# erikszasz/GaussianSplattingRegistration

Measured on AMD Instinct MI355X. Metric: Gaussians/sec through HEM level + ICP iters/sec, 2x5M-splat pair, higher is better.
Workload: dtype f32 (HEM) / f64 (ICP)

## Files before the change

### gaussiansplattingregistration_amd/_lib.py

```python
from __future__ import annotations

import ctypes as C
import os

_HERE = os.path.dirname(os.path.abspath(__file__))
LIB_PATH = os.environ.get("GSR_HIP_LIB") or os.path.join(_HERE, "csrc", "libgsr_hip.so")

GSR_OK = 0
GSR_E_INVALID = -1
GSR_E_HIP = -2
GSR_E_NO_DEVICE = -3
GSR_E_PRECONDITION = -4

GSR_RNG_GLIBC = 0
GSR_RNG_HASH = 1

GSR_ICP_ACC_LEN = 32

GSR_COMM_ID_BYTES = 128

GSR_DECOMP_REFERENCE = 0
GSR_DECOMP_EXACT = 1

ALLREDUCE_FN = C.CFUNCTYPE(C.c_int32, C.POINTER(C.c_double), C.c_int32, C.c_void_p)
# ... 75 lines not shown
    "gsr_normals_from_cov": (_i32, [_vp, _i64, _vp, _i32, _i32, _vp]),
    "gsr_normals_knn": (_i32, [_vp, _i64, _i32, _vp, _i32, _i32, _vp]),
    "gsr_cov_from_normals": (_i32, [_vp, _i64, _f64, _vp, _i32, _i32, _vp]),
    "gsr_decompose_cov": (_i32, [_vp, _i64, _i32, _vp, _vp, _vp, _i32, _i32, _vp]),
    "gsr_ply_unpack": (_i32, [_vp, _i64, _i32, C.POINTER(_i32), _i32, _vp, _vp, _vp, _vp, _vp, _vp, _vp, _i32, _vp]),
    "gsr_ply_pack": (_i32, [_vp, _vp, _vp, _vp, _vp, _vp, _i64, _i32, _vp, _i32, _vp]),
    "gsr_sh_rotation": (_i32, [_vp, _i32, _vp]),
    "gsr_model_transform": (_i32, [_vp, _i64, _i32, _i32, _vp, _vp, _vp, _vp, _vp, _vp, _vp, _vp, _i32, _i32, _vp]),
    "gsr_model_similarity": (_i32, [_vp, _i64, _i32, _i32, _vp, _vp, _vp, _vp, _vp, _vp, _vp, _vp, _vp, _vp, _i32, _i32, _vp]),
    "gsr_model_fuse": (_i32, [_vp, _vp, _i32, _vp, _vp, _vp, _vp, _i32, _i32, _vp]),
    "gsr_plane_score": (_i32, [_vp, _vp, _i64, _vp, _i32, _f32, _f32, _vp, _vp, C.POINTER(_i32), _i32, _i32, _vp]),
    "gsr_icp_solve": (_i32, [_vp, _i32, _vp, _vp]),
    "gsr_icp_get_centre": (_i32, [_vp, _vp]),
    "gsr_hybrid_search": (_i32, [_vp, _i64, _f64, _i32, _vp, _vp, _i32, _i32, _vp]),
    "gsr_fpfh": (_i32, [_vp, _vp, _i64, _f64, _i32, _vp, _i32, _i32, _vp]),
    "gsr_feature_match": (_i32, [_vp, _i64, _vp, _i64, _i32, _i32, _vp, C.POINTER(_i64), C.POINTER(_i32), _vp, _vp, _i32, _i32, _vp]),
    "gsr_ransac_correspondence": (_i32, [_vp, _i64, _vp, _i64, _vp, _vp, _vp, _i64, _vp, _vp, _i32, _i32, _vp]),
    "gsr_fgr_tuple_test": (_i32, [_vp, _i64, _vp, _i64, _vp, _i64, _vp, _vp, C.POINTER(_i64), C.POINTER(_i64), _i32, _i32, _vp]),
    "gsr_fgr_optimize": (_i32, [_vp, _i64, _vp, _i64, _vp, _i64, _vp, _vp, _i32, _i32, _vp]),
    "gsr_posegraph_optimize": (_i32, [_i32, _vp, _i32, _vp, _vp, _vp, _vp, _vp]),
    "gsr_raster_create": (_i32, [C.POINTER(_vp), _i32, _vp]),
    "gsr_raster_destroy": (_i32, [_vp]),
    "gsr_raster_render": (_i32, [_vp, _i64, _i32, _i32, _vp, _vp, _vp, _vp, _vp, C.POINTER(_f32), _f32, _f32, _f32, _f32, _i32, _i32, C.POINTER(_f32), _f32,
                                 _vp, _vp, _vp]),
    "gsr_raster_get_timing": (_i32, [_vp, C.POINTER(_f32)]),
    "gsr_image_metrics": (_i32, [_vp, _vp, _i32, _i32, _i32, C.POINTER(_f64), _i32, _vp]),
}
TEST_HOOKS = {
    "gsr_debug_logf": (_i32, [_vp, _i64, _vp, _i32]),
    "gsr_debug_kld": (_i32, [_vp, _vp, _vp, _vp, _i64, _vp, _i32]),
    "gsr_debug_kl_gate": (_i32, [_vp, _vp, _vp, _i64, _f32, _vp, _vp, _vp, _i32]),
    "gsr_debug_stage1": (_i32, [_vp, _vp, _vp, _vp, _i64, _f32, _vp, _vp, _vp, _vp, _vp, _vp, _i32]),
    "gsr_debug_ransac_sample": (_i32, [_u64, _i64, _i64, _i64, _i32, _vp]),
}

_lib = None


class HemLevelReport(C.Structure):
    _fields_ = [("offset_rows", C.c_int64), ("rows", C.c_int64), ("dropped", C.c_int64), ("rng_position", C.c_uint64),
                ("stats", C.c_int64 * 8), ("stats_ex", C.c_int64 * 8), ("phase_ms", C.c_float * 8), ("kernel_ms", C.c_float * 8)]


class IcpEntry(C.Structure):
    _fields_ = [("src_xyz", C.c_void_p), ("ns", C.c_int64), ("tgt_xyz", C.c_void_p), ("tgt_normals", C.c_void_p), ("nt", C.c_int64),
                ("max_corr", C.c_double), ("max_iter", C.c_int32), ("reserved", C.c_int32)]


class IcpEntryResult(C.Structure):
    _fields_ = [("init_T", C.c_double * 16), ("T", C.c_double * 16), ("fitness", C.c_double), ("inlier_rmse", C.c_double),
                ("iterations", C.c_int32), ("evaluations", C.c_int32), ("ms_build", C.c_float), ("ms_iters", C.c_float)]


class RansacParams(C.Structure):
    _fields_ = [("kind", C.c_int32), ("ransac_n", C.c_int32), ("max_corr", C.c_double), ("max_iteration", C.c_int64),
                ("confidence", C.c_double), ("seed", C.c_uint64), ("batch", C.c_int32), ("n_checkers", C.c_int32),
                ("checker_kind", C.c_int32 * 4), ("checker_param", C.c_double * 4)]


class RansacResult(C.Structure):
    _fields_ = [("T", C.c_double * 16), ("fitness", C.c_double), ("inlier_rmse", C.c_double), ("best_index", C.c_int64),
                ("n_evaluated", C.c_int64), ("n_valid", C.c_int64), ("exit_index", C.c_int64)]


class FgrOptions(C.Structure):
    _fields_ = [("division_factor", C.c_double), ("use_absolute_scale", C.c_int32), ("decrease_mu", C.c_int32),
# ... 74 lines not shown
```

### gaussiansplattingregistration_amd/csrc/gsr_test_hooks.h

```cpp
#ifndef GSR_TEST_HOOKS_H
#define GSR_TEST_HOOKS_H
#include <stdint.h>
#ifdef __cplusplus
extern "C" {
#endif
int32_t gsr_debug_logf(const float* x, int64_t n, float* out, int32_t device);
int32_t gsr_debug_kld(const float* child_mean, const float* child_cov6, const float* parent_mean,
                      const float* parent_cov6, int64_t n, float* out, int32_t device);
int32_t gsr_debug_kl_gate(const float* s2, const float* det_c, const float* det_p, int64_t n, float thr, uint8_t* reject,
                          float* fast_log, uint8_t* need_exact, int32_t device);
int32_t gsr_debug_stage1(const float* parent_mean, const float* parent_cov6, const float* child_mean, const float* child_cov6, int64_t n,
                         float kld_thr, uint8_t* parent_regular, uint8_t* child_regular, uint8_t* white, uint8_t* reject, float* T1,
                         uint8_t* clip_on, int32_t device);
int32_t gsr_debug_ransac_sample(uint64_t seed, int64_t k0, int64_t count, int64_t m, int32_t n, int32_t* out);
#ifdef __cplusplus
}
#endif
#endif
```

### gaussiansplattingregistration_amd/csrc/icp.hip

```cpp
#include "gsr_common.h"
#include "gsr_normals.h"
#include "gsr_solve.h"
#include "gsr_features.h"
#include "gsr_oneshot.h"
#include "gsr_prims.h"

#include <float.h>
#include <math.h>
#include <stdlib.h>
#include <string.h>
#include <vector>

namespace gsr {
#ifndef GSR_ICP_MERGE_BS
#define GSR_ICP_MERGE_BS 1024
#define GSR_ICP_MERGE_IPT 4
#endif
using icp_merge_cfg = rocprim::merge_sort_config<512, GSR_ICP_MERGE_BS, GSR_ICP_MERGE_IPT, 128, 128, 4>;
using icp_sort_cfg = rocprim::radix_sort_config<rocprim::default_config, icp_merge_cfg,
                                                rocprim::radix_sort_onesweep_config<rocprim::kernel_config<1024, 16>, rocprim::kernel_config<1024, 16>, 11,
                                                                                    rocprim::block_radix_rank_algorithm::match>>;

#ifndef ICP_CELL_FLOOR_DIV
#define ICP_CELL_FLOOR_DIV 64.0
#endif
struct IcpGrid {
    double ox, oy, oz, inv_c, c;
    double cx, cy, cz;
    int gx, gy, gz, ncells;
    int rings;
    double bx0, by0, bz0, bx1, by1, bz1;
};

__device__ __forceinline__ int icp_cell(double v, double o, double inv_c, int g) {
    double t = (v - o) * inv_c;
    t = fmin(fmax(t, 0.0), (double)(g - 1));
    return (int)t;
}

__global__ __launch_bounds__(256) void k_icp_bbox(int64_t n, const float* __restrict__ xyz, float* __restrict__ bbox_part) {
    float mn[3] = {FLT_MAX, FLT_MAX, FLT_MAX}, mx[3] = {-FLT_MAX, -FLT_MAX, -FLT_MAX};
    for (int64_t i = (int64_t)blockIdx.x * blockDim.x + threadIdx.x; i < n; i += (int64_t)gridDim.x * blockDim.x) {
        float x = xyz[3 * i], y = xyz[3 * i + 1], z = xyz[3 * i + 2];
        if (fabsf(x) <= FLT_MAX && fabsf(y) <= FLT_MAX && fabsf(z) <= FLT_MAX) {
            mn[0] = fminf(mn[0], x); mx[0] = fmaxf(mx[0], x);
            mn[1] = fminf(mn[1], y); mx[1] = fmaxf(mx[1], y);
            mn[2] = fminf(mn[2], z); mx[2] = fmaxf(mx[2], z);
        }
    }
    __shared__ float s_mn[4][3], s_mx[4][3];
    for (int k = 0; k < 3; ++k)
        for (int o = 32; o > 0; o >>= 1) { mn[k] = fminf(mn[k], __shfl_xor(mn[k], o)); mx[k] = fmaxf(mx[k], __shfl_xor(mx[k], o)); }
    if ((threadIdx.x & 63) == 0)
        for (int k = 0; k < 3; ++k) { s_mn[threadIdx.x >> 6][k] = mn[k]; s_mx[threadIdx.x >> 6][k] = mx[k]; }
    __syncthreads();
    if (threadIdx.x < 3) {
        const int k = threadIdx.x;
        float a = s_mn[0][k], b = s_mx[0][k];
        for (int w = 1; w < 4; ++w) { a = fminf(a, s_mn[w][k]); b = fmaxf(b, s_mx[w][k]); }
        bbox_part[6 * blockIdx.x + k] = a;
        bbox_part[6 * blockIdx.x + 3 + k] = b;
    }
}
__global__ __launch_bounds__(256) void k_icp_bbox_reduce(int nblocks, const float* __restrict__ part, float* __restrict__ bbox) {
// ... 120 lines not shown

struct ColorArgs {
    const double* t_int;
    const double* t_grad;
    const double* s_int;
    double sqrt_lg, sqrt_lp;
};

__device__ __forceinline__ void icp_scan_span(const int* __restrict__ cellStart, const float4* __restrict__ Tq, int first, int last,
                                              double px, double py, double pz, double& bd, int& best, unsigned& best_i) {
    const int s = cellStart[first], e = cellStart[last + 1];
    for (int j = s; j < e; ++j) {
        const float4 q = Tq[j];
        const double dx = px - (double)q.x, dy = py - (double)q.y, dz = pz - (double)q.z;
        const double d2 = dx * dx + dy * dy + dz * dz;
        const unsigned qi = __float_as_uint(q.w);
        if (d2 < bd || (d2 == bd && qi < best_i)) { bd = d2; best = j; best_i = qi; }
    }
}

__device__ __forceinline__ double icp_slab_dist(double v, double o, double c, int k, double eps, int g) {
    const double lo = o + (double)k * c, hi = o + (double)(k + 1) * c;
    const double d = ((v < lo && k > 0) ? lo - v : ((v > hi && k < g - 1) ? v - hi : 0.0)) * 0.999999999 - eps;
    return d > 0.0 ? d : 0.0;
}

__device__ __forceinline__ void icp_consider(const float4 q, int j, double px, double py, double pz, double& bd, int& best, unsigned& best_i) {
    const double dx = px - (double)q.x, dy = py - (double)q.y, dz = pz - (double)q.z;
    const double d2 = dx * dx + dy * dy + dz * dz;
    const unsigned qi = __float_as_uint(q.w);
    if (d2 < bd || (d2 == bd && qi < best_i)) { bd = d2; best = j; best_i = qi; }
}

#define ICP_BLOCK_CROWDED 24
#ifndef ICP_ROW_BATCH
#define ICP_ROW_BATCH 4
#endif
template <int BLOCK>
__device__ __forceinline__ int icp_nearest(const IcpGrid& g, const int* __restrict__ cellStart,
                                           const float4* __restrict__ Tq, double px, double py, double pz, double& best_d2,
                                           double bound2 = 1.0 / 0.0) {
    int best = -1;
    unsigned best_i = 0xffffffffu;
    double bd = bound2;
    if (!(px == px) || !(py == py) || !(pz == pz)) { best_d2 = 1.0 / 0.0; return -1; }
    {
        const double ex = fmax(fmax(g.bx0 - px, px - g.bx1), 0.0), ey = fmax(fmax(g.by0 - py, py - g.by1), 0.0), ez = fmax(fmax(g.bz0 - pz, pz - g.bz1), 0.0);
        if ((ex * ex + ey * ey + ez * ez) * 0.999999999 >= bound2) { best_d2 = bound2; return -1; }
    }
    const int cx = icp_cell(px, g.ox, g.inv_c, g.gx), cy = icp_cell(py, g.oy, g.inv_c, g.gy), cz = icp_cell(pz, g.oz, g.inv_c, g.gz);
    const double eps = 1e-13 * (fabs(px) + fabs(py) + fabs(pz) + fabs(g.ox) + fabs(g.oy) + fabs(g.oz) + g.c * (double)(g.gx + g.gy + g.gz));
    int r0 = 0;
    if (BLOCK == 1 && g.rings >= 1) {
        int rs[9], re[9];
        const int xa = cx - 1 > 0 ? cx - 1 : 0, xb = cx + 1 < g.gx - 1 ? cx + 1 : g.gx - 1;
#pragma unroll
        for (int t = 0; t < 9; ++t) {
            const int z = cz + t / 3 - 1, y = cy + t % 3 - 1;
            const bool ok = z >= 0 && z < g.gz && y >= 0 && y < g.gy;
            const int rowbase = ok ? (z * g.gy + y) * g.gx : 0;
            rs[t] = ok ? cellStart[rowbase + xa] : 0;
            re[t] = ok ? cellStart[rowbase + xb + 1] : 0;
        }
        {
        constexpr int order9[9] = {4, 1, 3, 5, 7, 0, 2, 6, 8};
#pragma unroll
        for (int tt = 0; tt < 9; ++tt) {
            const int t = order9[tt];
            if (t != 4 && re[t] - rs[t] > ICP_BLOCK_CROWDED) {
                const double dzb = icp_slab_dist(pz, g.oz, g.c, cz + t / 3 - 1, eps, g.gz), dyb = icp_slab_dist(py, g.oy, g.c, cy + t % 3 - 1, eps, g.gy);
                if (dzb * dzb + dyb * dyb > bd) continue;
            }
            for (int j = rs[t]; j < re[t]; j += ICP_ROW_BATCH) {
                const int l = re[t] - 1;
                int jj[ICP_ROW_BATCH];
                float4 qq[ICP_ROW_BATCH];
#pragma unroll
                for (int b = 0; b < ICP_ROW_BATCH; ++b) { jj[b] = j + b < l ? j + b : l; qq[b] = Tq[jj[b]]; }
#pragma unroll
                for (int b = 0; b < ICP_ROW_BATCH; ++b) icp_consider(qq[b], jj[b], px, py, pz, bd, best, best_i);
            }
        }
        }
    }
    if (BLOCK && g.rings >= 1) {
        double reach = 1.0 / 0.0;
        if (cx - 1 > 0) reach = fmin(reach, px - (g.ox + (double)(cx - 1) * g.c));
        if (cx + 1 < g.gx - 1) reach = fmin(reach, (g.ox + (double)(cx + 2) * g.c) - px);
        if (cy - 1 > 0) reach = fmin(reach, py - (g.oy + (double)(cy - 1) * g.c));
        if (cy + 1 < g.gy - 1) reach = fmin(reach, (g.oy + (double)(cy + 2) * g.c) - py);
        if (cz - 1 > 0) reach = fmin(reach, pz - (g.oz + (double)(cz - 1) * g.c));
        if (cz + 1 < g.gz - 1) reach = fmin(reach, (g.oz + (double)(cz + 2) * g.c) - pz);
        reach = reach * 0.999999999 - eps;
        reach = reach > 0.0 ? reach : 0.0;
        if (bd < reach * reach) { best_d2 = bd; return best; }
        r0 = 2;
    }
    for (int r = r0; r <= g.rings; ++r) {
        for (int dz = -r; dz <= r; ++dz) {
            const int z = cz + dz;
            if (z < 0 || z >= g.gz) continue;
            const int adz = dz < 0 ? -dz : dz;
            const double dzb = icp_slab_dist(pz, g.oz, g.c, z, eps, g.gz);
            for (int dy = -r; dy <= r; ++dy) {
                const int y = cy + dy;
                if (y < 0 || y >= g.gy) continue;
                const int ady = dy < 0 ? -dy : dy;
                const double dyb = icp_slab_dist(py, g.oy, g.c, y, eps, g.gy);
                const double rem = bd - dyb * dyb - dzb * dzb;
                if (rem < 0.0) continue;
                int xlo = 0, xhi = g.gx - 1;
                if (rem < 1e300) {
                    const double hx = (double)(sqrtf((float)rem) * 1.0001f) + eps + 1e-30;
                    xlo = icp_cell(px - hx, g.ox, g.inv_c, g.gx);
                    xhi = icp_cell(px + hx, g.ox, g.inv_c, g.gx);
// ... 36 lines not shown
    IcpRange r;
    r.row = L < nb ? L : -1;
    r.lo = (int64_t)L * ppb;
    r.hi = r.lo + ppb < ns ? r.lo + ppb : ns;
    return r;
}

struct IcpState;
__device__ __forceinline__ bool icp_state_done(const IcpState* st);
__device__ __forceinline__ void icp_state_T(const IcpState* st, double T[12]);

template <bool FROM_STATE, int BLOCK>
__global__ __launch_bounds__(256) void k_icp_nn(int64_t ns, const float* __restrict__ src, Xform X, const IcpState* __restrict__ st,
                                                IcpGrid g, const int* __restrict__ cellStart, const float4* __restrict__ Tq,
                                                double max_corr2, int* __restrict__ nn_j, int nb_logical) {
    double T[12];
    if (FROM_STATE) {
        if (icp_state_done(st)) return;
        icp_state_T(st, T);
    } else {
#pragma unroll
        for (int i = 0; i < 12; ++i) T[i] = X.m[i];
    }
    const IcpRange rg = icp_block_range(ns, nb_logical < 0 ? -nb_logical : nb_logical, nb_logical > 0);
    if (rg.row < 0) return;
    for (int64_t i = rg.lo + threadIdx.x; i < rg.hi; i += blockDim.x) {
        const double x = (double)src[3 * i], y = (double)src[3 * i + 1], z = (double)src[3 * i + 2];
        const double px = T[0] * x + T[1] * y + T[2] * z + T[3];
        const double py = T[4] * x + T[5] * y + T[6] * z + T[7];
        const double pz = T[8] * x + T[9] * y + T[10] * z + T[11];
        double d2;
        const int j = icp_nearest<BLOCK>(g, cellStart, Tq, px, py, pz, d2, max_corr2);
        nn_j[i] = (j >= 0 && d2 < max_corr2) ? j : -1;
    }
}

__device__ __forceinline__ double icp_weight(int loss, double k, double r) {
    switch (loss) {
        case GSR_LOSS_TUKEY: { double t = fmin(1.0, fabs(r) / k); double u = 1.0 - t * t; return u * u; }
        case GSR_LOSS_CAUCHY: { double t = r / k; return 1.0 / (1.0 + t * t); }
        case GSR_LOSS_GM: { double t = k + r * r; return k / (t * t); }
        case GSR_LOSS_HUBER: { double e = fabs(r); return k / fmax(e, k); }
        default: return 1.0;
    }
}

__host__ __device__ static void sym_eig3(double a00, double a01, double a02, double a11, double a12, double a22, double V[3][3], double lam[3]) {
    double A[3][3] = {{a00, a01, a02}, {a01, a11, a12}, {a02, a12, a22}};
    for (int i = 0; i < 3; ++i) for (int j = 0; j < 3; ++j) V[i][j] = i == j ? 1.0 : 0.0;
    for (int sweep = 0; sweep < 30; ++sweep) {
        const double off = A[0][1] * A[0][1] + A[0][2] * A[0][2] + A[1][2] * A[1][2];
        const double dg = A[0][0] * A[0][0] + A[1][1] * A[1][1] + A[2][2] * A[2][2];
        if (!(off > 1e-40 * dg)) break;
#pragma unroll
        for (int p = 0; p < 2; ++p)
#pragma unroll
            for (int q = p + 1; q < 3; ++q) {
                if (A[p][q] == 0.0) continue;
                const double theta = (A[q][q] - A[p][p]) / (2.0 * A[p][q]);
                const double t = (theta >= 0 ? 1.0 : -1.0) / (fabs(theta) + sqrt(theta * theta + 1.0));
                const double c = 1.0 / sqrt(t * t + 1.0), sn = t * c;
#pragma unroll
                for (int k = 0; k < 3; ++k) { const double x = A[k][p], y = A[k][q]; A[k][p] = c * x - sn * y; A[k][q] = sn * x + c * y; }
#pragma unroll
                for (int k = 0; k < 3; ++k) { const double x = A[p][k], y = A[q][k]; A[p][k] = c * x - sn * y; A[q][k] = sn * x + c * y; }
#pragma unroll
// ... 615 lines not shown
    icp_step_solve(&s_x[0][0], s_st, st);
}

__global__ __launch_bounds__(1024) void k_icp_reduce(int nblocks, const double* __restrict__ partials, const IcpState* __restrict__ st,
                                                     double* __restrict__ out) {
    const int lane = threadIdx.x & 63, wv = threadIdx.x >> 6;
    const bool done = st->done != 0;
    for (int k = wv; k < GSR_ICP_ACC_LEN; k += 16) {
        double s = 0.0;
        if (!done)
            for (int b = lane; b < nblocks; b += 64) s += partials[(int64_t)b * GSR_ICP_ACC_LEN + k];
        for (int o = 32; o > 0; o >>= 1) s += __shfl_xor(s, o);
        if (lane == 0) out[k] = s;
    }
}

}

using namespace gsr;

struct gsr_icp_ctx {
    int device = 0;
    hipStream_t stream = nullptr;
    IcpGrid grid;
    bool have_target = false, have_normals = false, have_source = false;
    int64_t nt = 0, ns = 0, ns_global = 0;
    double max_corr = 0;
    DevBuf src_raw, src_order, state, nn_j, Tc, Sc, stage_cov, Ti, Tg, Si;
    bool have_tcov = false, have_scov = false, have_tcol = false, have_scol = false;
    double lambda_geometric = 0.968;
    bool src_sorted = false;
    bool device_loop = true;
    bool block_search = true;
    bool xcd_ranges = true;
    gsr_comm* comm = nullptr;
    PinnedBlock host_rb;
    unsigned long long rb_seq = 0;
    int nn_kernel = -1;
    int nn_mode() const { return nn_kernel >= 0 ? (nn_kernel ? 2 : 0) : (ns >= 400000 ? 2 : 0); }
    double cell_target = 2.0;
    DevBuf hist;
    bool robust_box = false;
    bool robust_allowed = true;
    DevBuf bbox, keys, idx, skeys, order, cellStart, Tq, Tn, stage_xyz, stage_nrm, src, partials, acc_dev, rocprim_tmp, corr_idx, corr_d2;
    gsr_allreduce_fn allreduce = nullptr;
    void* allreduce_user = nullptr;
    gsr_allreduce_dev64_fn allreduce_dev = nullptr;
    void* allreduce_dev_user = nullptr;
    Event e0, e1, eb0, eb1;
    bool defer_sync = false;
    bool build_pending = false;
    float ms_build = 0, ms_iter = 0;
    int n_iter_kernels = 0;
    int max_cells = 1 << 25;
    int nblocks = 768;
    ~gsr_icp_ctx() { (void)hipSetDevice(device); }
};

namespace {

inline int icp_blocks(int64_t ns, int cap) {
    if (ns <= 0) return 1;
    const int64_t ppb = ((ns + cap - 1) / cap + 255) / 256 * 256;
    return (int)((ns + ppb - 1) / ppb);
}
inline int nn_grid1(int64_t ns) { return icp_blocks(ns, 16384); }
// ... 117 lines not shown
static int32_t icp_fetch(gsr_icp_ctx* c, const void* dev, void* out, size_t bytes) {
    hipStream_t st = c->stream;
    unsigned* const host_rb = c->host_rb.as<unsigned>();
    if (!host_rb || bytes > 1024 || (bytes & 3)) {
        GSR_HIP(hipMemcpyAsync(out, dev, bytes, hipMemcpyDeviceToHost, st));
        GSR_HIP(hipStreamSynchronize(st));
        return GSR_OK;
    }
    const unsigned long long seq = ++c->rb_seq;
    unsigned long long* flag = reinterpret_cast<unsigned long long*>(host_rb + 256);
    hipLaunchKernelGGL(k_icp_publish, dim3(1), dim3(64), 0, st, (const unsigned*)dev, (int)(bytes >> 2), host_rb, flag, seq);
    GSR_HIP(hipGetLastError());
    GSR_TRY(wait_host_flag(st, flag, seq, true));
    memcpy(out, (const void*)host_rb, bytes);
    return GSR_OK;
}

int32_t gsr_icp_create(gsr_icp_ctx** out, int32_t device, void* stream) {
    if (!out) return fail(GSR_E_INVALID, "gsr_icp_create: out is NULL");
    *out = nullptr;
    int ndev = 0;
    if (hipGetDeviceCount(&ndev) != hipSuccess || ndev <= 0)
        return fail(GSR_E_NO_DEVICE, "gsr_icp_create: no HIP device visible (this backend has no CPU fallback)");
    if (device < 0 || device >= ndev) return fail(GSR_E_INVALID, "gsr_icp_create: device %d out of range", device);
    GSR_HIP(hipSetDevice(device));
    gsr_icp_ctx* c = new gsr_icp_ctx();
    c->device = device;
    c->stream = (hipStream_t)stream;
    if (c->e0.create() != hipSuccess || c->e1.create() != hipSuccess || c->eb0.create() != hipSuccess || c->eb1.create() != hipSuccess) {
        delete c; return fail(GSR_E_HIP, "hipEventCreate failed");
    }
    if (const char* e = getenv("GSR_ICP_DEVICE_LOOP")) c->device_loop = atoi(e) != 0;
    if (const char* e = getenv("GSR_ICP_BLOCK_SEARCH")) c->block_search = atoi(e) != 0;
    if (const char* e = getenv("GSR_ICP_XCD")) c->xcd_ranges = atoi(e) != 0;
    if (const char* e = getenv("GSR_ICP_ROBUST_BOX")) c->robust_allowed = atoi(e) != 0;
    if (const char* e = getenv("GSR_ICP_BLOCKS")) { int v = atoi(e); if (v >= 1 && v <= 65536) c->nblocks = v; }
    bool poll = true;
    if (const char* e = getenv("GSR_ICP_RB_POLL")) poll = atoi(e) != 0;
    if (!poll || c->host_rb.alloc(1024 + 64) != hipSuccess) (void)hipGetLastError();
    if (const char* e = getenv("GSR_ICP_NN_KERNEL")) c->nn_kernel = atoi(e);
    if (const char* e = getenv("GSR_ICP_CELL_TARGET")) { double v = atof(e); if (v > 0.01 && v < 1000) c->cell_target = v; }
    if (const char* e = getenv("GSR_ICP_MAX_CELLS")) { int v = atoi(e); if (v >= 1024) c->max_cells = v; }
    *out = c;
    return GSR_OK;
}

int32_t gsr_icp_destroy(gsr_icp_ctx* c) {
    delete c;
    return GSR_OK;
}

int32_t gsr_icp_set_target(gsr_icp_ctx* c, const float* xyz, const double* normals, int64_t n, double max_corr, int32_t on_device) {
    if (!c) return fail(GSR_E_INVALID, "gsr_icp_set_target: NULL context");
    if (!(max_corr > 0)) return fail(GSR_E_PRECONDITION, "max_correspondence_distance must be > 0 (got %g)", max_corr);
    if (n <= 0 || !xyz) return fail(GSR_E_PRECONDITION, "gsr_icp_set_target: empty target cloud");
    if (n >= ((int64_t)1 << 31) - 1) return fail(GSR_E_INVALID, "gsr_icp_set_target: n too large");
    GSR_HIP(hipSetDevice(c->device));
    hipStream_t st = c->stream;
    GSR_HIP(hipEventRecord(c->eb0, st));
    const float* dxyz = xyz;
    const double* dnrm = normals;
    if (!on_device) {
        GSR_TRY(c->stage_xyz.reserve((size_t)n * 12));
        GSR_HIP(hipMemcpyAsync(c->stage_xyz.p, xyz, (size_t)n * 12, hipMemcpyHostToDevice, st));
        dxyz = c->stage_xyz.as<float>();
        if (normals) {
// ... 14 lines not shown
    GSR_TRY(icp_fetch(c, c->bbox.p, hb, 13 * 4));
    const float raw_box[6] = {hb[0], hb[1], hb[2], hb[3], hb[4], hb[5]};
    c->robust_box = hb[12] != 0.0f && c->robust_allowed;
    if (c->robust_box) {
        GSR_HIP(hipMemsetAsync(c->hist.p, 0, 3 * ICP_HIST_BINS * 4, st));
        hipLaunchKernelGGL(k_icp_hist, dim3(nbb > 512 ? 512 : nbb), dim3(256), 0, st, n, dxyz, c->bbox.as<float>() + 6, c->hist.as<unsigned>());
        hipLaunchKernelGGL(k_icp_trim, dim3(1), dim3(64), 0, st, c->hist.as<unsigned>(), c->bbox.as<float>() + 6, c->bbox.as<float>(), c->bbox.as<float>() + 12);
        GSR_TRY(icp_fetch(c, c->bbox.p, hb, 6 * 4));
    }
    double mn[3], mx[3];
    for (int k = 0; k < 3; ++k) { mn[k] = hb[k]; mx[k] = hb[3 + k]; }
    IcpGrid g;
    if (!(mx[0] >= mn[0])) { mn[0] = mn[1] = mn[2] = 0; mx[0] = mx[1] = mx[2] = 0; }
    double cell;
    {
        const double ex = mx[0] - mn[0], ey = mx[1] - mn[1], ez = mx[2] - mn[2];
        const double emax = fmax(ex, fmax(ey, ez)), eps = emax * 1e-6 + 1e-30;
        cell = cbrt((ex + eps) * (ey + eps) * (ez + eps) * c->cell_target / (double)n);
        if (!(cell > 0)) cell = max_corr;
        if (cell < max_corr / ICP_CELL_FLOOR_DIV) cell = max_corr / ICP_CELL_FLOOR_DIV;
    }
    GSR_TRY(c->keys.reserve(n * 4)); GSR_TRY(c->idx.reserve(n * 4)); GSR_TRY(c->skeys.reserve(n * 4)); GSR_TRY(c->order.reserve(n * 4));
    for (;;) {
        double fx = floor((mx[0] - mn[0]) / cell) + 1, fy = floor((mx[1] - mn[1]) / cell) + 1, fz = floor((mx[2] - mn[2]) / cell) + 1;
        if (fx * fy * fz <= (double)c->max_cells) { g.gx = (int)fx; g.gy = (int)fy; g.gz = (int)fz; break; }
        cell *= 1.2599210498948732;
    }
    g.ox = mn[0]; g.oy = mn[1]; g.oz = mn[2];
    g.c = cell; g.inv_c = 1.0 / cell;
    g.cx = 0.5 * (mn[0] + mx[0]); g.cy = 0.5 * (mn[1] + mx[1]); g.cz = 0.5 * (mn[2] + mx[2]);
    g.ncells = g.gx * g.gy * g.gz;
    g.rings = (int)ceil(max_corr / cell);
    if (g.rings < 1) g.rings = 1;
    g.bx0 = raw_box[0]; g.by0 = raw_box[1]; g.bz0 = raw_box[2]; g.bx1 = raw_box[3]; g.by1 = raw_box[4]; g.bz1 = raw_box[5];
    if (!(raw_box[3] >= raw_box[0])) { g.bx0 = g.by0 = g.bz0 = -1.0 / 0.0; g.bx1 = g.by1 = g.bz1 = 1.0 / 0.0; }
    hipLaunchKernelGGL(k_icp_keys, dim3(stride_grid(n)), dim3(256), 0, st, n, dxyz, g, c->keys.as<unsigned>(), c->idx.as<unsigned>());
    int bits = 1;
    while (bits < 32 && ((int64_t)1 << bits) < g.ncells) ++bits;
    GSR_TRY(sort_pairs_by_key<icp_sort_cfg>(c->rocprim_tmp, st, c->keys.as<unsigned>(), c->skeys.as<unsigned>(), c->idx.as<unsigned>(),
                                            c->order.as<unsigned>(), (size_t)n, 0u, (unsigned)bits));
    GSR_TRY(c->cellStart.reserve(((size_t)g.ncells + 1) * 4));
    hipLaunchKernelGGL(k_icp_cell_starts, dim3(stride_grid(n)), dim3(256), 0, st, n, c->skeys.as<unsigned>(), (int64_t)g.ncells, c->cellStart.as<int>());
    c->grid = g;
    GSR_TRY(c->Tq.reserve((size_t)n * 16));
    if (normals) GSR_TRY(c->Tn.reserve((size_t)n * 24));
    hipLaunchKernelGGL(k_icp_gather_target, dim3(stride_grid(n)), dim3(256), 0, st, n, c->order.as<unsigned>(), dxyz, dnrm,
                       c->Tq.as<float4>(), normals ? c->Tn.as<double>() : (double*)nullptr);
    GSR_HIP(hipEventRecord(c->eb1, st));
    if (c->defer_sync) c->build_pending = true;
    else {
        GSR_HIP(hipStreamSynchronize(st));
        (void)hipEventElapsedTime(&c->ms_build, c->eb0, c->eb1);
        c->build_pending = false;
    }
    GSR_HIP(hipGetLastError());
    c->nt = n; c->max_corr = max_corr; c->have_target = true; c->have_normals = normals != nullptr;
    c->have_tcov = false; c->have_scov = false; c->have_tcol = false; c->have_scol = false;
    c->have_source = false;
    return GSR_OK;
}

int32_t gsr_icp_set_source(gsr_icp_ctx* c, const float* xyz, int64_t n, int32_t on_device) {
    if (!c) return fail(GSR_E_INVALID, "gsr_icp_set_source: NULL context");
    if (n < 0 || (n > 0 && !xyz)) return fail(GSR_E_PRECONDITION, "gsr_icp_set_source: empty source cloud");
    if (n >= ((int64_t)1 << 31) - 1) return fail(GSR_E_INVALID, "gsr_icp_set_source: n too large");
    GSR_HIP(hipSetDevice(c->device));
    hipStream_t st = c->stream;
    GSR_TRY(c->src.reserve((size_t)(n > 0 ? n : 1) * 12));
// ... 208 lines not shown
        return GSR_OK;
    }
    double T[16], acc[GSR_ICP_ACC_LEN], update[16];
    memcpy(T, init_T, sizeof(T));
    GSR_TRY(run_accumulate(c, T, kind, loss, k, acc, true));
    const double nsg = (double)(c->ns_global > 0 ? c->ns_global : c->ns);
    double fit = acc[0] > 0 ? acc[0] / nsg : 0.0, rmse = acc[0] > 0 ? sqrt(acc[1] / acc[0]) : 0.0;
    int it = 0;
    for (; it < max_iter; ++it) {
        const double ctr[3] = {c->grid.cx, c->grid.cy, c->grid.cz};
        estimate_update(ctr, kind, acc, update);
        mat4_mul(update, T, T);
        GSR_TRY(run_accumulate(c, T, kind, loss, k, acc, true));
        const double fit2 = acc[0] > 0 ? acc[0] / nsg : 0.0, rmse2 = acc[0] > 0 ? sqrt(acc[1] / acc[0]) : 0.0;
        const bool stop = fabs(fit - fit2) < rel_fitness && fabs(rmse - rmse2) < rel_rmse;
        fit = fit2; rmse = rmse2;
        if (stop) { ++it; break; }
    }
    memcpy(out_T, T, sizeof(T));
    if (fitness) *fitness = fit;
    if (inlier_rmse) *inlier_rmse = rmse;
    if (iterations) *iterations = it;
    return GSR_OK;
}

int32_t gsr_icp_correspondences(gsr_icp_ctx* c, const double* T, int64_t* idx, double* d2) {
    if (!c || !T || !idx || !d2) return fail(GSR_E_INVALID, "gsr_icp_correspondences: NULL argument");
    if (!c->have_target || !c->have_source) return fail(GSR_E_INVALID, "icp: target and source must be set first");
    GSR_HIP(hipSetDevice(c->device));
    GSR_TRY(c->corr_idx.reserve((size_t)c->ns * 8)); GSR_TRY(c->corr_d2.reserve((size_t)c->ns * 8));
    Xform X;
    for (int i = 0; i < 12; ++i) X.m[i] = T[i];
    GSR_TRY(c->nn_j.reserve((size_t)c->ns * 4));
    launch_icp_nn<false>(c, c->stream, X, (const IcpState*)nullptr, c->max_corr * c->max_corr, false);
    hipLaunchKernelGGL(k_icp_correspond, dim3(stride_grid(c->ns)), dim3(256), 0, c->stream, c->ns, c->src.as<float>(), X, c->nn_j.as<int>(),
                       c->Tq.as<float4>(), c->src_sorted ? c->src_order.as<unsigned>() : (const unsigned*)nullptr, c->corr_idx.as<int64_t>(),
                       c->corr_d2.as<double>());
    GSR_HIP(hipMemcpyAsync(idx, c->corr_idx.p, (size_t)c->ns * 8, hipMemcpyDeviceToHost, c->stream));
    GSR_HIP(hipMemcpyAsync(d2, c->corr_d2.p, (size_t)c->ns * 8, hipMemcpyDeviceToHost, c->stream));
    GSR_HIP(hipStreamSynchronize(c->stream));
    return GSR_OK;
}

int32_t gsr_icp_information(gsr_icp_ctx* c, const double* T, double* info36, int64_t* n_corr) {
    if (!c || !T || !info36) return fail(GSR_E_INVALID, "gsr_icp_information: NULL argument");
    if (!c->have_target || !c->have_source) return fail(GSR_E_INVALID, "gsr_icp_information: target and source must be set first");
    if (c->comm || c->allreduce || c->allreduce_dev)
        return fail(GSR_E_INVALID, "gsr_icp_information: one process, one GPU -- this context has a communicator or an all-reduce callback installed "
                                   "(the sums of a source shard are not the pair's information matrix)");
    for (int i = 0; i < 16; ++i)
        if (!(fabs(T[i]) <= DBL_MAX)) return fail(GSR_E_INVALID, "gsr_icp_information: T[%d] is not finite", i);
    GSR_HIP(hipSetDevice(c->device));
    hipStream_t st = c->stream;
    Xform X;
    for (int i = 0; i < 12; ++i) X.m[i] = T[i];
    const int nb = icp_blocks(c->ns, c->nblocks);
    GSR_TRY(c->partials.reserve((size_t)nb * GSR_ICP_ACC_LEN * 8));
    GSR_TRY(c->acc_dev.reserve(GSR_ICP_ACC_LEN * 8));
    GSR_HIP(hipMemsetAsync(c->partials.p, 0, (size_t)nb * GSR_ICP_ACC_LEN * 8, st));
    const double mc2 = c->max_corr * c->max_corr;
    const int* nnj = nullptr;
    if (c->nn_mode()) {
        GSR_TRY(c->nn_j.reserve((size_t)c->ns * 4));
        launch_icp_nn<false>(c, st, X, (const IcpState*)nullptr, mc2, false);
        nnj = c->nn_j.as<int>();
    }
    hipLaunchKernelGGL(k_icp_information, dim3(nb), dim3(256), 0, st, c->ns, c->src.as<float>(), X, c->grid, c->cellStart.as<int>(), nnj, c->Tq.as<float4>(),
                       mc2, c->partials.as<double>());
    hipLaunchKernelGGL(k_icp_finalize, dim3(ICP_INFO_NACC), dim3(64), 0, st, nb, c->partials.as<double>(), c->acc_dev.as<double>());
    double a[ICP_INFO_NACC];
    GSR_HIP(hipMemcpyAsync(a, c->acc_dev.p, sizeof(a), hipMemcpyDeviceToHost, st));
    GSR_HIP(hipStreamSynchronize(st));
    const double n = a[0], mx = a[1], my = a[2], mz = a[3];
    const double nxy = 0.0 - a[5], nxz = 0.0 - a[6], nyz = 0.0 - a[8];
    const double A[3][3] = {{a[7] + a[9], nxy, nxz}, {nxy, a[4] + a[9], nyz}, {nxz, nyz, a[4] + a[7]}};
    const double Mx[3][3] = {{0.0, 0.0 - mz, my}, {mz, 0.0, 0.0 - mx}, {0.0 - my, mx, 0.0}};
// ... 249 lines not shown
```

Before: 577.8 million.

## Add f32 screening pass to ICP nearest-neighbour search with certified error bounds

Adds a first pass to the ICP nearest-neighbour search that computes distances in f32 and tracks the best and second-best candidates. If a rigorous rounding-error bound shows the f32 winner cannot be overtaken, that single candidate is confirmed in f64 and the full f64 scan is skipped. Otherwise the existing f64 search runs. The aim is to replace most f64 distance arithmetic, which is slow on this GPU, with f32. The risk is that ambiguous points pay for both passes, and the extra registers may lower occupancy. A debug hook is added to report the screen's decisions.

Result: slower. 569.7 million (-1.4%).

```diff
diff --git a/gaussiansplattingregistration_amd/_lib.py b/gaussiansplattingregistration_amd/_lib.py
--- a/gaussiansplattingregistration_amd/_lib.py
+++ b/gaussiansplattingregistration_amd/_lib.py
@@ -131,6 +131,7 @@
     "gsr_debug_kl_gate": (_i32, [_vp, _vp, _vp, _i64, _f32, _vp, _vp, _vp, _i32]),
     "gsr_debug_stage1": (_i32, [_vp, _vp, _vp, _vp, _i64, _f32, _vp, _vp, _vp, _vp, _vp, _vp, _i32]),
     "gsr_debug_ransac_sample": (_i32, [_u64, _i64, _i64, _i64, _i32, _vp]),
+    "gsr_debug_icp_search": (_i32, [_vp, _vp, _i32, _i32, _vp, _vp, _vp, _vp, _vp, C.POINTER(_i64)]),
 }
 
 _lib = None
diff --git a/gaussiansplattingregistration_amd/csrc/gsr_test_hooks.h b/gaussiansplattingregistration_amd/csrc/gsr_test_hooks.h
--- a/gaussiansplattingregistration_amd/csrc/gsr_test_hooks.h
+++ b/gaussiansplattingregistration_amd/csrc/gsr_test_hooks.h
@@ -13,6 +13,9 @@
                          float kld_thr, uint8_t* parent_regular, uint8_t* child_regular, uint8_t* white, uint8_t* reject, float* T1,
                          uint8_t* clip_on, int32_t device);
 int32_t gsr_debug_ransac_sample(uint64_t seed, int64_t k0, int64_t count, int64_t m, int32_t n, int32_t* out);
+struct gsr_icp_ctx;
+int32_t gsr_debug_icp_search(struct gsr_icp_ctx* c, const double* T, int32_t block, int32_t screen, int64_t* idx, double* d2, float* m1,
+                             float* m2, uint8_t* decided, int64_t* n_undecided);
 #ifdef __cplusplus
 }
 #endif
diff --git a/gaussiansplattingregistration_amd/csrc/icp.hip b/gaussiansplattingregistration_amd/csrc/icp.hip
--- a/gaussiansplattingregistration_amd/csrc/icp.hip
+++ b/gaussiansplattingregistration_amd/csrc/icp.hip
@@ -29,7 +29,9 @@
     double cx, cy, cz;
     int gx, gy, gz, ncells;
     int rings;
+    int screen;
     double bx0, by0, bz0, bx1, by1, bz1;
+    double bmax;
 };
 
 __device__ __forceinline__ int icp_cell(double v, double o, double inv_c, int g) {
@@ -216,6 +218,14 @@
     if (d2 < bd || (d2 == bd && qi < best_i)) { bd = d2; best = j; best_i = qi; }
 }
 
+__device__ __forceinline__ double icp_screen_err(float d, double delta) {
+    return 2.0 * ((double)sqrtf(d) * 1.000001) * delta + delta * delta + 0x1p-21 * (double)d + 1e-37;
+}
+__device__ __forceinline__ double icp_screen_delta(const IcpGrid& g, double px, double py, double pz) {
+    return 3.4641016151377553 * 0x1p-24 * fmax(fmax(fmax(fabs(px), fabs(py)), fabs(pz)), g.bmax);
+}
+struct IcpScreenInfo { float m1, m2; int state; };
+
 #define ICP_BLOCK_CROWDED 24
 #ifndef ICP_ROW_BATCH
 #define ICP_ROW_BATCH 4
@@ -223,7 +233,7 @@
 template <int BLOCK>
 __device__ __forceinline__ int icp_nearest(const IcpGrid& g, const int* __restrict__ cellStart,
                                            const float4* __restrict__ Tq, double px, double py, double pz, double& best_d2,
-                                           double bound2 = 1.0 / 0.0) {
+                                           double bound2 = 1.0 / 0.0, IcpScreenInfo* info = nullptr) {
     int best = -1;
     unsigned best_i = 0xffffffffu;
     double bd = bound2;
@@ -246,8 +256,54 @@
             rs[t] = ok ? cellStart[rowbase + xa] : 0;
             re[t] = ok ? cellStart[rowbase + xb + 1] : 0;
         }
-        {
         constexpr int order9[9] = {4, 1, 3, 5, 7, 0, 2, 6, 8};
+        bool decided = false;
+        if (g.screen) {
+            const float pfx = (float)px, pfy = (float)py, pfz = (float)pz;
+            const double delta = icp_screen_delta(g, px, py, pz);
+            const float inf = __builtin_inff();
+            float m1 = inf, m2 = inf;
+            int j1 = 0;
+#pragma unroll
+            for (int tt = 0; tt < 9; ++tt) {
+                const int t = order9[tt];
+                if (t != 4 && re[t] - rs[t] > ICP_BLOCK_CROWDED) {
+                    const double dzb = icp_slab_dist(pz, g.oz, g.c, cz + t / 3 - 1, eps, g.gz), dyb = icp_slab_dist(py, g.oy, g.c, cy + t % 3 - 1, eps, g.gy);
+                    const double ub = m1 < inf ? fmin(bound2, (double)m1 + icp_screen_err(m1, delta)) : bound2;
+                    if (dzb * dzb + dyb * dyb > ub) continue;
+                }
+                for (int j = rs[t]; j < re[t]; j += ICP_ROW_BATCH) {
+                    const int l = re[t] - 1;
+                    float4 qq[ICP_ROW_BATCH];
+#pragma unroll
+                    for (int b = 0; b < ICP_ROW_BATCH; ++b) qq[b] = Tq[j + b < l ? j + b : l];
+#pragma unroll
+                    for (int b = 0; b < ICP_ROW_BATCH; ++b) {
+                        float sx = pfx - qq[b].x, sy = pfy - qq[b].y, sz = pfz - qq[b].z;
+                        asm("" : "+v"(sx), "+v"(sy), "+v"(sz));
+                        float d = __builtin_fmaf(sz, sz, __builtin_fmaf(sy, sy, sx * sx));
+                        d = j + b > l ? inf : d;
+                        m2 = fminf(m2, fmaxf(d, m1));
+                        j1 = d < m1 ? j + b : j1;
+                        m1 = fminf(m1, d);
+                    }
+                }
+            }
+            int rows = 0;
+#pragma unroll
+            for (int t = 0; t < 9; ++t) rows += re[t] - rs[t];
+            if (rows == 0) decided = true;
+            else if (m1 < inf) {
+                const double hi1 = (double)m1 + icp_screen_err(m1, delta);
+                const double lo2 = m2 < inf ? (double)m2 - icp_screen_err(m2, delta) : 3e38;
+                if (hi1 < lo2) {
+                    decided = true;
+                    icp_consider(Tq[j1], j1, px, py, pz, bd, best, best_i);
+                }
+            }
+            if (info) { info->m1 = m1; info->m2 = m2; info->state = decided ? 1 : 2; }
+        }
+        if (!decided) {
 #pragma unroll
         for (int tt = 0; tt < 9; ++tt) {
             const int t = order9[tt];
@@ -367,6 +423,29 @@
         double d2;
         const int j = icp_nearest<BLOCK>(g, cellStart, Tq, px, py, pz, d2, max_corr2);
         nn_j[i] = (j >= 0 && d2 < max_corr2) ? j : -1;
+    }
+}
+
+template <int BLOCK>
+__global__ __launch_bounds__(256) void k_icp_search_debug(int64_t ns, const float* __restrict__ src, Xform X, IcpGrid g, const int* __restrict__ cellStart,
+                                                          const float4* __restrict__ Tq, double max_corr2, const unsigned* __restrict__ src_order,
+                                                          int64_t* __restrict__ idx, double* __restrict__ d2_out, float* __restrict__ m1, float* __restrict__ m2,
+                                                          unsigned char* __restrict__ decided, unsigned long long* __restrict__ n_undecided) {
+    for (int64_t i = (int64_t)blockIdx.x * blockDim.x + threadIdx.x; i < ns; i += (int64_t)gridDim.x * blockDim.x) {
+        const double x = (double)src[3 * i], y = (double)src[3 * i + 1], z = (double)src[3 * i + 2];
+        const double px = X.m[0] * x + X.m[1] * y + X.m[2] * z + X.m[3];
+        const double py = X.m[4] * x + X.m[5] * y + X.m[6] * z + X.m[7];
+        const double pz = X.m[8] * x + X.m[9] * y + X.m[10] * z + X.m[11];
+        IcpScreenInfo info = {__builtin_inff(), __builtin_inff(), 0};
+        double d2;
+        const int j = icp_nearest<BLOCK>(g, cellStart, Tq, px, py, pz, d2, max_corr2, &info);
+        const bool ok = j >= 0 && d2 < max_corr2;
+        const int64_t o = src_order ? (int64_t)src_order[i] : i;
+        idx[o] = ok ? (int64_t)__float_as_uint(Tq[j].w) : -1;
+        d2_out[o] = ok ? d2 : 1.0 / 0.0;
+        m1[o] = info.m1; m2[o] = info.m2;
+        decided[o] = info.state == 1 ? 1 : 0;
+        if (info.state == 2) atomicAdd(n_undecided, 1ull);
     }
 }
 
@@ -1048,6 +1127,7 @@
     bool src_sorted = false;
     bool device_loop = true;
     bool block_search = true;
+    bool f32_screen = true;
     bool xcd_ranges = true;
     gsr_comm* comm = nullptr;
     PinnedBlock host_rb;
@@ -1231,6 +1311,7 @@
     }
     if (const char* e = getenv("GSR_ICP_DEVICE_LOOP")) c->device_loop = atoi(e) != 0;
     if (const char* e = getenv("GSR_ICP_BLOCK_SEARCH")) c->block_search = atoi(e) != 0;
+    if (const char* e = getenv("GSR_ICP_F32_SCREEN")) c->f32_screen = atoi(e) != 0;
     if (const char* e = getenv("GSR_ICP_XCD")) c->xcd_ranges = atoi(e) != 0;
     if (const char* e = getenv("GSR_ICP_ROBUST_BOX")) c->robust_allowed = atoi(e) != 0;
     if (const char* e = getenv("GSR_ICP_BLOCKS")) { int v = atoi(e); if (v >= 1 && v <= 65536) c->nblocks = v; }
@@ -1311,8 +1392,10 @@
     g.ncells = g.gx * g.gy * g.gz;
     g.rings = (int)ceil(max_corr / cell);
     if (g.rings < 1) g.rings = 1;
+    g.screen = c->f32_screen ? 1 : 0;
     g.bx0 = raw_box[0]; g.by0 = raw_box[1]; g.bz0 = raw_box[2]; g.bx1 = raw_box[3]; g.by1 = raw_box[4]; g.bz1 = raw_box[5];
     if (!(raw_box[3] >= raw_box[0])) { g.bx0 = g.by0 = g.bz0 = -1.0 / 0.0; g.bx1 = g.by1 = g.bz1 = 1.0 / 0.0; }
+    g.bmax = fmax(fmax(fmax(fabs(g.bx0), fabs(g.bx1)), fmax(fabs(g.by0), fabs(g.by1))), fmax(fabs(g.bz0), fabs(g.bz1)));
     hipLaunchKernelGGL(k_icp_keys, dim3(stride_grid(n)), dim3(256), 0, st, n, dxyz, g, c->keys.as<unsigned>(), c->idx.as<unsigned>());
     int bits = 1;
     while (bits < 32 && ((int64_t)1 << bits) < g.ncells) ++bits;
@@ -1597,6 +1680,50 @@
     return GSR_OK;
 }
 
+int32_t gsr_debug_icp_search(gsr_icp_ctx* c, const double* T, int32_t block, int32_t screen, int64_t* idx, double* d2, float* m1, float* m2,
+                             uint8_t* decided, int64_t* n_undecided) {
+    if (!c || !T || !idx || !d2 || !m1 || !m2 || !decided || !n_undecided) return fail(GSR_E_INVALID, "gsr_debug_icp_search: NULL argument");
+    if (!c->have_target || !c->have_source) return fail(GSR_E_INVALID, "gsr_debug_icp_search: target and source must be set first");
+    GSR_HIP(hipSetDevice(c->device));
+    hipStream_t st = c->stream;
+    const size_t n = (size_t)c->ns;
+    *n_undecided = 0;
+    if (n == 0) return GSR_OK;
+    DevBuf out;
+    GSR_TRY(out.reserve(n * 25 + 8));
+    char* const base = out.as<char>();
+    int64_t* const d_idx = (int64_t*)base;
+    double* const d_d2 = (double*)(base + n * 8);
+    float* const d_m1 = (float*)(base + n * 16);
+    float* const d_m2 = (float*)(base + n * 20);
+    unsigned long long* const d_cnt = (unsigned long long*)(base + n * 24);
+    unsigned char* const d_dec = (unsigned char*)(base + n * 24 + 8);
+    GSR_HIP(hipMemsetAsync(d_cnt, 0, 8, st));
+    Xform X;
+    for (int i = 0; i < 12; ++i) X.m[i] = T[i];
+    IcpGrid g = c->grid;
+    g.screen = screen ? 1 : 0;
+    const unsigned* order = c->src_sorted ? c->src_order.as<unsigned>() : (const unsigned*)nullptr;
+    const double mc2 = c->max_corr * c->max_corr;
+    if (block)
+        hipLaunchKernelGGL(k_icp_search_debug<1>, dim3(stride_grid(c->ns)), dim3(256), 0, st, c->ns, c->src.as<float>(), X, g, c->cellStart.as<int>(),
+                           c->Tq.as<float4>(), mc2, order, d_idx, d_d2, d_m1, d_m2, d_dec, d_cnt);
+    else
+        hipLaunchKernelGGL(k_icp_search_debug<0>, dim3(stride_grid(c->ns)), dim3(256), 0, st, c->ns, c->src.as<float>(), X, g, c->cellStart.as<int>(),
+                           c->Tq.as<float4>(), mc2, order, d_idx, d_d2, d_m1, d_m2, d_dec, d_cnt);
+    GSR_HIP(hipGetLastError());
+    unsigned long long cnt = 0;
+    GSR_HIP(hipMemcpyAsync(idx, d_idx, n * 8, hipMemcpyDeviceToHost, st));
+    GSR_HIP(hipMemcpyAsync(d2, d_d2, n * 8, hipMemcpyDeviceToHost, st));
+    GSR_HIP(hipMemcpyAsync(m1, d_m1, n * 4, hipMemcpyDeviceToHost, st));
+    GSR_HIP(hipMemcpyAsync(m2, d_m2, n * 4, hipMemcpyDeviceToHost, st));
+    GSR_HIP(hipMemcpyAsync(decided, d_dec, n, hipMemcpyDeviceToHost, st));
+    GSR_HIP(hipMemcpyAsync(&cnt, d_cnt, 8, hipMemcpyDeviceToHost, st));
+    GSR_HIP(hipStreamSynchronize(st));
+    *n_undecided = (int64_t)cnt;
+    return GSR_OK;
+}
+
 int32_t gsr_icp_information(gsr_icp_ctx* c, const double* T, double* info36, int64_t* n_corr) {
     if (!c || !T || !info36) return fail(GSR_E_INVALID, "gsr_icp_information: NULL argument");
     if (!c->have_target || !c->have_source) return fail(GSR_E_INVALID, "gsr_icp_information: target and source must be set first");
```

## Flatten 3x3 row walk into single loop with batch spill across rows

Applied to the files above, without the earlier changes.

Replaces the nested per-row loop of the nine neighbouring cell rows in the block nearest-neighbour search with a single flattened loop. The non-empty row ranges are staged in shared memory, and leftover batch slots can spill into the next short row, so fewer ICP_ROW_BATCH lanes are wasted on clamped duplicates and warp divergence across rows drops. Crowded rows are still pruned by slab distance. Separately, the correspondence entry point now enables block search when it is configured and the grid has enough rings. This adds shared memory use (a 9x256 int2 array) and assumes a block size of at most 256.

Result: no change. 580.5 million before, 577.1 million after (-0.6%).

```diff
diff --git a/gaussiansplattingregistration_amd/csrc/icp.hip b/gaussiansplattingregistration_amd/csrc/icp.hip
--- a/gaussiansplattingregistration_amd/csrc/icp.hip
+++ b/gaussiansplattingregistration_amd/csrc/icp.hip
@@ -235,7 +235,8 @@
     const int cx = icp_cell(px, g.ox, g.inv_c, g.gx), cy = icp_cell(py, g.oy, g.inv_c, g.gy), cz = icp_cell(pz, g.oz, g.inv_c, g.gz);
     const double eps = 1e-13 * (fabs(px) + fabs(py) + fabs(pz) + fabs(g.ox) + fabs(g.oy) + fabs(g.oz) + g.c * (double)(g.gx + g.gy + g.gz));
     int r0 = 0;
-    if (BLOCK == 1 && g.rings >= 1) {
+    if constexpr (BLOCK == 1) if (g.rings >= 1) {
+        __shared__ int2 s_rows[9][256];
         int rs[9], re[9];
         const int xa = cx - 1 > 0 ? cx - 1 : 0, xb = cx + 1 < g.gx - 1 ? cx + 1 : g.gx - 1;
 #pragma unroll
@@ -246,25 +247,59 @@
             rs[t] = ok ? cellStart[rowbase + xa] : 0;
             re[t] = ok ? cellStart[rowbase + xb + 1] : 0;
         }
-        {
         constexpr int order9[9] = {4, 1, 3, 5, 7, 0, 2, 6, 8};
+        unsigned rows = 0;
+        int nrows = 0;
 #pragma unroll
         for (int tt = 0; tt < 9; ++tt) {
             const int t = order9[tt];
-            if (t != 4 && re[t] - rs[t] > ICP_BLOCK_CROWDED) {
-                const double dzb = icp_slab_dist(pz, g.oz, g.c, cz + t / 3 - 1, eps, g.gz), dyb = icp_slab_dist(py, g.oy, g.c, cy + t % 3 - 1, eps, g.gy);
-                if (dzb * dzb + dyb * dyb > bd) continue;
+            if (re[t] > rs[t]) {
+                s_rows[nrows][threadIdx.x] = make_int2(rs[t], re[t]);
+                rows |= 1u << tt;
+                ++nrows;
             }
-            for (int j = rs[t]; j < re[t]; j += ICP_ROW_BATCH) {
-                const int l = re[t] - 1;
-                int jj[ICP_ROW_BATCH];
-                float4 qq[ICP_ROW_BATCH];
-#pragma unroll
-                for (int b = 0; b < ICP_ROW_BATCH; ++b) { jj[b] = j + b < l ? j + b : l; qq[b] = Tq[jj[b]]; }
-#pragma unroll
-                for (int b = 0; b < ICP_ROW_BATCH; ++b) icp_consider(qq[b], jj[b], px, py, pz, bd, best, best_i);
+        }
+        int j = 0, e = 0, jn = 0, en = 0, off = 0, lim = 0, k = 0;
+        bool spill = false;
+        if (nrows > 0) { const int2 r = s_rows[0][threadIdx.x]; jn = r.x; en = r.y; k = 1; }
+        for (;;) {
+            while (j >= e && jn < en) {
+                bool skip = false;
+                if (en - jn > ICP_BLOCK_CROWDED) {
+                    const int tt = __ffs((int)rows) - 1;
+                    if (tt != 0) {
+                        const int t = (int)((0x86207531u >> (4 * (tt - 1))) & 15u);
+                        const double dzb = icp_slab_dist(pz, g.oz, g.c, cz + t / 3 - 1, eps, g.gz), dyb = icp_slab_dist(py, g.oy, g.c, cy + t % 3 - 1, eps, g.gy);
+                        skip = dzb * dzb + dyb * dyb > bd;
+                    }
+                }
+                rows &= rows - 1;
+                j = jn + (spill ? j - e : 0);
+                j = (skip || j > en) ? en : j;
+                e = en;
+                jn = en = 0;
+                if (k < nrows) { const int2 r = s_rows[k][threadIdx.x]; jn = r.x; en = r.y; ++k; }
+#ifdef ICP_WALK_NOSPILL
+                spill = false;
+#else
+                spill = jn < en && en - jn <= ICP_BLOCK_CROWDED;
+#endif
+                off = spill ? jn - e : 0;
+                lim = spill ? en - 1 : e - 1;
             }
-        }
+            if (j >= e) break;
+            int jj[ICP_ROW_BATCH];
+            float4 qq[ICP_ROW_BATCH];
+#pragma unroll
+            for (int b = 0; b < ICP_ROW_BATCH; ++b) {
+                int i = j + b;
+                if (i >= e) { i += off; i = i < lim ? i : lim; }
+                jj[b] = i;
+                qq[b] = Tq[i];
+            }
+#pragma unroll
+            for (int b = 0; b < ICP_ROW_BATCH; ++b) icp_consider(qq[b], jj[b], px, py, pz, bd, best, best_i);
+            j += ICP_ROW_BATCH;
         }
     }
     if (BLOCK && g.rings >= 1) {
@@ -1587,7 +1622,7 @@
     Xform X;
     for (int i = 0; i < 12; ++i) X.m[i] = T[i];
     GSR_TRY(c->nn_j.reserve((size_t)c->ns * 4));
-    launch_icp_nn<false>(c, c->stream, X, (const IcpState*)nullptr, c->max_corr * c->max_corr, false);
+    launch_icp_nn<false>(c, c->stream, X, (const IcpState*)nullptr, c->max_corr * c->max_corr, c->block_search && c->grid.rings >= 2);
     hipLaunchKernelGGL(k_icp_correspond, dim3(stride_grid(c->ns)), dim3(256), 0, c->stream, c->ns, c->src.as<float>(), X, c->nn_j.as<int>(),
                        c->Tq.as<float4>(), c->src_sorted ? c->src_order.as<unsigned>() : (const unsigned*)nullptr, c->corr_idx.as<int64_t>(),
                        c->corr_d2.as<double>());
```
